# satoken/dafs

Measured on AMD Instinct MI355X. Metric: seq-pairs/sec (all-pairs ProbCons pair-HMM posteriors + sparse rows + sim), higher is better.
Workload: dtype f32; 1 GPU; N=128 L~150 synthetic random RNA (seed 12345), 8128 pairs; align_model=ProbCons, kernel=k_pairhmm3<G=32,W=6> x 4064 waves

## Files before the change

dafs_amd/capi.py:

```python
import ctypes as C
import os

import numpy as np

_HERE = os.path.dirname(os.path.abspath(__file__))
LIB_PATH = os.environ.get("DAFS_HIP_LIB") or os.path.join(_HERE, "libdafs_hip.so")

NONE = 0xFFFFFFFF
ALIGN_PROBCONS, ALIGN_CONTRALIGN = 0, 1
E_OVERFLOW = -5


class DafsHipError(RuntimeError):
    pass


def _load():
    if not os.path.exists(LIB_PATH):
        raise DafsHipError(
            "libdafs_hip.so is not built (%s). Run `python -m dafs_amd.build`; there is no CPU fallback." % LIB_PATH)
    return C.CDLL(LIB_PATH)


lib = _load()
# ... 209 lines not shown
_nodes_advance = _sig("dafs_hip_nodes_advance", C.c_int, [C.c_void_p, C.c_uint32, C.c_void_p, C.POINTER(DDParams), C.c_uint32, C.c_void_p])
_nodes_round = _sig("dafs_hip_nodes_round", C.c_int, [C.c_void_p, C.c_uint32, C.POINTER(NodeInput), C.c_void_p, C.c_uint32, C.c_void_p,
                                                      C.POINTER(DDParams), C.c_uint32, C.c_uint32, C.c_void_p, C.c_void_p])
_nodes_result = _sig("dafs_hip_nodes_result", C.c_int, [C.c_void_p, C.c_uint32, C.POINTER(NodeOutput)])
_nodes_close = _sig("dafs_hip_nodes_close", C.c_int, [C.c_void_p])
_nodes_memory = _sig("dafs_hip_nodes_memory", C.c_int, [C.c_void_p, C.POINTER(C.c_uint64), C.POINTER(C.c_uint64), C.POINTER(C.c_uint64)])
_nodes_demotions = _sig("dafs_hip_nodes_demotions", C.c_int, [C.c_void_p, C.POINTER(C.c_uint32)])
_update_basepairing = _sig("dafs_hip_update_basepairing", C.c_int, [C.c_void_p, C.c_uint32, C.c_uint32, C.c_void_p, C.c_void_p, C.c_void_p, C.c_void_p])
_consensus_structure = _sig("dafs_hip_consensus_structure", C.c_int,
                            [C.c_void_p, C.c_uint32, C.c_uint32, C.c_void_p, C.c_void_p, C.c_float, C.c_void_p,
                             C.POINTER(C.c_float), C.c_void_p])
_structure_levels_bytes = _sig("dafs_host_structure_levels_bytes", C.c_uint64, [C.c_uint32, C.c_uint32])
_consensus_structures_levels = _sig("dafs_hip_consensus_structures_levels", C.c_int,
                                    [C.c_void_p, C.c_uint32, C.c_void_p, C.c_void_p, C.c_void_p, C.c_void_p, C.c_uint32, C.c_void_p,
                                     C.c_void_p, C.c_void_p, C.c_void_p])
_structure_auto_bytes = _sig("dafs_host_structure_auto_bytes", C.c_uint64, [C.c_uint32, C.c_uint32, C.c_uint32])
_consensus_structures_auto = _sig("dafs_hip_consensus_structures_auto", C.c_int,
                                  [C.c_void_p, C.c_uint32, C.c_void_p, C.c_void_p, C.c_void_p, C.c_void_p, C.c_uint32, C.c_uint32]
                                  + [C.c_void_p] * 10)
_consensus_structures = _sig("dafs_hip_consensus_structures", C.c_int,
                             [C.c_void_p, C.c_uint32, C.c_void_p, C.c_void_p, C.c_void_p, C.c_void_p, C.c_float, C.c_void_p, C.c_void_p])
_alignment_reliability = _sig("dafs_hip_alignment_reliability", C.c_int,
                              [C.c_void_p, C.c_uint32, C.c_uint32, C.c_void_p, C.c_void_p, C.c_void_p, C.c_int, C.c_int] + [C.c_void_p] * 5)
_alignment_reliabilities = _sig("dafs_hip_alignment_reliabilities", C.c_int,
                                [C.c_void_p, C.c_uint32] + [C.c_void_p] * 6 + [C.c_int, C.c_int] + [C.c_void_p] * 5)
_alignment_covariation = _sig("dafs_hip_alignment_covariation", C.c_int,
                              [C.c_void_p, C.c_uint32, C.c_uint32, C.c_void_p, C.c_void_p, C.c_uint32, C.c_uint64] + [C.c_void_p] * 11)
_alignment_covariation_null = _sig("dafs_hip_alignment_covariation_null", C.c_int,
                                   [C.c_void_p, C.c_uint32, C.c_uint32, C.c_void_p, C.c_void_p, C.c_uint32, C.c_uint64, C.c_int, C.c_void_p,
                                    C.c_void_p] + [C.c_void_p] * 11)
_covariation_null_alignment = _sig("dafs_hip_covariation_null_alignment", C.c_int,
                                   [C.c_void_p, C.c_uint32, C.c_uint32, C.c_void_p, C.c_int, C.c_void_p, C.c_void_p, C.c_uint64, C.c_uint32,
                                    C.c_void_p])
COV_NULLS = ("shuffle", "tree")
_alignment_identity = _sig("dafs_hip_alignment_identity", C.c_int,
                           [C.c_void_p, C.c_uint32, C.c_uint32, C.c_void_p, C.c_void_p, C.c_void_p, C.c_double] + [C.c_void_p] * 7)
_alignment_weights = _sig("dafs_hip_alignment_weights", C.c_int, [C.c_void_p, C.c_uint32, C.c_uint32, C.c_void_p, C.c_void_p, C.c_void_p])


class CompareOut(C.Structure):
    _fields_ = [(k, C.c_void_p) for k in ("residues", "shared", "refp", "testp", "sps", "ppv", "total", "score", "k", "m", "colref", "colshared",
                                         "reproduced", "tc", "pair_shared", "pair_refp", "pair_testp", "pp_count", "tp", "nref", "ntest", "ss_total")]


_alignment_compare = _sig("dafs_hip_alignment_compare", C.c_int, [C.c_void_p, C.c_uint32, C.c_uint32, C.c_uint32] + [C.c_void_p] * 7 + [C.POINTER(CompareOut)])
_compare_refusal = _sig("dafs_host_compare_refusal", C.c_char_p, [C.c_int])
CMP_NEEDS_REF, CMP_NEEDS_COMPARE, CMP_NO_PAIRWISE, CMP_NEEDS_MERGED, CMP_TOO_MANY_ROWS = range(5)
_compare_match = _sig("dafs_host_compare_match", C.c_int, [C.c_uint32, C.POINTER(C.c_char_p), C.c_uint32, C.POINTER(C.c_char_p)] + [C.c_void_p] * 3)
_seed_pp = _sig("dafs_host_seed_pp", C.c_int, [C.c_char_p, C.c_size_t, C.POINTER(C.c_uint32), C.POINTER(C.c_int), C.POINTER(C.c_void_p)])
_compare_table = _sig("dafs_host_compare_table", C.c_int, [C.c_uint32, C.POINTER(C.c_char_p)] + [C.c_uint32] * 4 + [C.c_void_p] * 10 + [C.POINTER(C.c_void_p)])
_compare_columns_table = _sig("dafs_host_compare_columns_table", C.c_int, [C.c_uint32] + [C.c_void_p] * 4 + [C.POINTER(C.c_void_p)])
_compare_matrix_table = _sig("dafs_host_compare_matrix_table", C.c_int, [C.c_uint32, C.POINTER(C.c_char_p)] + [C.c_void_p] * 3 + [C.POINTER(C.c_void_p)])
_nr_select = _sig("dafs_host_nr_select", C.c_int, [C.c_uint32] + [C.c_void_p] * 5)
_ali_code = _sig("dafs_host_ali_code", C.c_uint8, [C.c_char])
_identity_summary = _sig("dafs_host_identity_summary", C.c_int, [C.c_uint32, C.c_void_p, C.c_void_p, C.c_void_p])
_identity_table = _sig("dafs_host_identity_table", C.c_int, [C.c_uint32, C.c_uint32, _strs] + [C.c_void_p] * 6 + [_text])
_identity_matrix_table = _sig("dafs_host_identity_matrix_table", C.c_int, [C.c_uint32, _strs] + [C.c_void_p] * 3 + [_text])
_stockholm_weights = _sig("dafs_host_stockholm_weights", C.c_int, [C.c_char_p, C.c_uint32, _strs, C.c_void_p, _text])
_stockholm_nr = _sig("dafs_host_stockholm_nr", C.c_int, [C.c_char_p, C.c_uint32, _strs, C.c_void_p, C.c_uint32, C.c_double, _text])
_alistat_refusal = _sig("dafs_host_alistat_refusal", C.c_char_p, [C.c_int])
NO_PAIRWISE, NR_NEEDS_MERGED, NR_THRESHOLD, TOO_MANY_ROWS = range(4)
_newick = _sig("dafs_host_newick", C.c_int, [C.c_uint32, _strs, C.c_void_p, C.c_void_p, C.c_void_p, _text])
_newick_support = _sig("dafs_host_newick_support", C.c_int, [C.c_uint32, _strs] + [C.c_void_p] * 4 + [C.c_uint32, _text])
_support_table = _sig("dafs_host_support_table", C.c_int, [C.c_uint32, _strs] + [C.c_void_p] * 3 + [C.c_uint32, C.c_uint64, C.c_int, _text])
_phylogeny_refusal = _sig("dafs_host_phylogeny_refusal", C.c_char_p, [C.c_int])
(PHY_NO_PAIRWISE, PHY_NO_SEED_EACH, PHY_TOO_MANY_ROWS, PHY_MODEL_NEEDS_TREE, PHY_UNKNOWN_MODEL, PHY_COV_TREE_NEEDS_NULL,
 PHY_UNKNOWN_COV_TREE) = range(7)
_bootstrap_refusal = _sig("dafs_host_bootstrap_refusal", C.c_char_p, [C.c_int])
BOOT_NEEDS_TREE, BOOT_COUNT, BOOT_NEEDS_REPLICATES, BOOT_NO_COLUMN = range(4)
_seed_table_nearest = _sig("dafs_host_seed_table_nearest", C.c_int, [C.c_uint32, _strs] + [C.c_void_p] * 8 + [_strs, C.c_void_p, _text])
_allgather_fn = C.CFUNCTYPE(C.c_int, C.c_void_p, C.c_void_p, C.c_void_p, C.c_size_t, C.c_void_p)
_phase1_sharded = _sig("dafs_hip_phase1_sharded", C.c_int, [C.c_void_p, C.c_uint32, C.c_uint32, C.c_int, C.c_float, C.c_float, C.c_float,
                                                           C.c_int, C.c_float, _allgather_fn, C.c_void_p])


class StageTime(C.Structure):
    _fields_ = [("kernel", C.c_char_p), ("ms", C.c_double), ("longest_ms", C.c_double), ("launches", C.c_uint32)]


_stage_timing = _sig("dafs_hip_stage_timing", C.c_int, [C.c_void_p, C.c_int])
_stage_report = _sig("dafs_hip_stage_report", C.c_int, [C.c_void_p, C.POINTER(StageTime), C.c_uint32, C.POINTER(C.c_uint32)])
pairhmm_plan = _sig("dafs_hipk_pairhmm_plan", C.c_int, [C.c_uint32, C.c_uint32, C.c_uint32, C.POINTER(PairhmmPlan)])
pairhmm3_launch = _sig("dafs_hipk_pairhmm3_launch", C.c_int, [C.POINTER(Pairhmm3Args), C.POINTER(PairhmmPlan), C.c_void_p])
pairhmm3_default_model = _sig("dafs_hip_pairhmm3_default_model", None, [C.POINTER(Pairhmm3Model)])
pairhmm5_plan = _sig("dafs_hipk_pairhmm5_plan", C.c_int, [C.c_uint32, C.c_uint32, C.c_uint32, C.POINTER(PairhmmPlan)])
pairhmm5_launch = _sig("dafs_hipk_pairhmm5_launch", C.c_int, [C.POINTER(Pairhmm5Args), C.POINTER(PairhmmPlan), C.c_void_p])
pairhmm5_default_model = _sig("dafs_hip_pairhmm5_default_model", None, [C.POINTER(Pairhmm5Model)])
residue_code = _sig("dafs_hip_residue_code", C.c_uint8, [C.c_char])
dd_node_plan = _sig("dafs_hipk_dd_node_plan", C.c_int, [C.c_uint32, C.c_uint32, C.POINTER(DdNodePlan)])
dd_lds_words = _sig("dafs_hipk_dd_lds_words", C.c_uint32, [C.c_uint32, C.c_uint32, C.c_uint32, C.c_uint32, C.c_int])


def check(rc):
    if rc != 0:
        raise DafsHipError("%s (code %d; hip: %s)" % (_strerror(rc).decode(), rc, _last_error().decode()))


def _allgather_callback(allgather, failures):
    def cb(user, send, recv, nbytes, stream):
        try:
            allgather(send, recv, nbytes)
        except BaseException as e:
            failures.append(e)
            return 1
        return 0
    return _allgather_fn(cb)


def encode(seq):
    b = seq.encode() if isinstance(seq, str) else bytes(seq)
    table = np.array([residue_code(bytes([i])) for i in range(256)], dtype=np.uint8)
    return table[np.frombuffer(b, dtype=np.uint8)]


_COV_CODE = np.array([_cov_code(bytes([i])) for i in range(256)], np.uint8)


def encode_alignment(rows):
    rows = [r.encode("latin-1") if isinstance(r, str) else bytes(r) for r in rows]
    if not rows or any(len(r) != len(rows[0]) for r in rows):
        raise ValueError("encode_alignment: at least one row, all of one length")
    return _COV_CODE[np.frombuffer(b"".join(rows), np.uint8)].reshape(len(rows), len(rows[0]))


_ALI_CODE = np.array([_ali_code(bytes([i])) for i in range(256)], np.uint8)


def encode_cells(rows):
    rows = [r.encode("latin-1") if isinstance(r, str) else bytes(r) for r in rows]
    if not rows or any(len(r) != len(rows[0]) for r in rows):
        raise ValueError("encode_cells: at least one row, all of one length")
    cell = _ALI_CODE[np.frombuffer(b"".join(rows), np.uint8)].reshape(len(rows), len(rows[0]))
    if (cell == 255).any():
        r, c = np.argwhere(cell == 255)[0]
        raise ValueError("encode_cells: row %d, column %d holds neither a letter nor a gap" % (r + 1, c + 1))
    return cell


def _cells(rows, who):
    if isinstance(rows, np.ndarray):
        if rows.ndim != 2 or rows.dtype.kind not in "iu":
            raise ValueError("%s: rows are text rows or a 2-D integer array of cells" % who)
        if rows.size and (rows.min() < 0 or rows.max() > 255):
            raise ValueError("%s: cells must fit a byte (the library refuses a code above 5)" % who)
        return np.ascontiguousarray(rows, np.uint8)
    return encode_cells(rows)


def _byte_mask(mask, size, who, what):
    if mask is None:
        return None
    mask = np.ascontiguousarray(np.asarray(mask) != 0, np.uint8)
    if mask.shape != (size,):
        raise ValueError("%s: %s" % (who, what))
    return mask


def alistat_refusal(which):
    return _alistat_refusal(which).decode()


class Identity:

    def bit(self, r, s):
        return bool((int(self.red[r, s // 32]) >> (s % 32)) & 1)

# ... 1136 lines not shown
```

dafs_amd/csrc/pair_sweeps.h:

```cpp
#pragma once
#include <hip/hip_runtime.h>
#include <stdint.h>
#include <stdlib.h>
#include "../../include/dafs_hip.h"
#include "hip_util.h"

namespace dafs {

__device__ __forceinline__ int dpp_row_shr1(int fill, int v) { return __builtin_amdgcn_update_dpp(fill, v, 0x111, 0xF, 0xF, false); }
__device__ __forceinline__ int dpp_row_shl1(int fill, int v) { return __builtin_amdgcn_update_dpp(fill, v, 0x101, 0xF, 0xF, false); }
__device__ __forceinline__ int dpp_wave_shr1(int fill, int v) { return __builtin_amdgcn_update_dpp(fill, v, 0x138, 0xF, 0xF, false); }
__device__ __forceinline__ int dpp_wave_shl1(int fill, int v) { return __builtin_amdgcn_update_dpp(fill, v, 0x130, 0xF, 0xF, false); }

template <int G>
__device__ __forceinline__ int shift_up1(int v, int fill, int t) {
  if constexpr (G == 16) return dpp_row_shr1(fill, v);
  const int r = dpp_wave_shr1(fill, v);
  if constexpr (G == 64) return r;
  return t == 0 ? fill : r;
}
template <int G>
__device__ __forceinline__ float shift_up1(float v, float fill, int t) {
  return __int_as_float(shift_up1<G>(__float_as_int(v), __float_as_int(fill), t));
}
template <int G>
__device__ __forceinline__ int shift_down1(int v, int fill, int t) {
  if constexpr (G == 16) return dpp_row_shl1(fill, v);
  const int r = dpp_wave_shl1(fill, v);
  if constexpr (G == 64) return r;
  return t == G - 1 ? fill : r;
}
template <int G>
__device__ __forceinline__ float shift_down1(float v, float fill, int t) {
  return __int_as_float(shift_down1<G>(__float_as_int(v), __float_as_int(fill), t));
}

template <int G, int W>
__device__ __forceinline__ int pair_width(int L2) {
  if constexpr (W == 1) return 1;
  int m = L2;
#pragma unroll
  for (int o = G; o < 64; o <<= 1) m = max(m, __shfl_xor(m, o));
  m = __builtin_amdgcn_readfirstlane(m);
  return (m + 1 <= G * (W - 1)) ? W - 1 : W;
}

template <int WR>
struct pair_rec {
  static constexpr int Q = (2 + WR + 3) / 4;
  static constexpr int D = 4 * Q;
};
template <int G, int W, int WR, bool dense, bool staged, class Args, class Post>
__device__ __forceinline__ bool pair_finish(const Args& a, float* __restrict__ slab, float* __restrict__ list, int list_cap, uint32_t* __restrict__ s_rowptr,
                                            uint2* __restrict__ stage, int E, int lane, int t, int g, int L1, int L2, int nsteps, bool act, uint32_t task,
                                            float th, Post post) {
  const int tlast = (L2 >= 0 ? L2 : 0) / WR;
  const int j0 = t * WR;
  typedef uint32_t u32x4 __attribute__((ext_vector_type(4)));
  const __amdgpu_buffer_rsrc_t list_rs = __builtin_amdgcn_make_buffer_rsrc((void*)list, 0, list_cap * 256, 0x00020000);
  constexpr uint32_t NO_RECORD = 0x80000000u;
  int colcnt[WR];
  float simv = 0.0f;
  uint32_t nnz = 0;
  int slab_nrec = 0;
  {
    float pdp[WR];
    int ptr[WR];
#pragma unroll
    for (int c = 0; c < WR; ++c) { pdp[c] = 0.0f; ptr[c] = 0; colcnt[c] = 0; }
    float lastdp = 0.0f, dgdp = 0.0f;
    int lasttr = 0, dgtr = 0, lastcnt = 0;
    uint32_t rowacc = 0;
    if (t == G - 1) s_rowptr[0] = 0;
    int nrec = 0;
    bool ovf = false;
    float sva[WR], svb[WR];
#pragma unroll
    for (int c = 0; c < WR; ++c) sva[c] = slab[c * 64 + lane];
#pragma unroll
    for (int c = 0; c < WR; ++c) svb[c] = slab[(W + c) * 64 + lane];
#pragma unroll
    for (int c = 0; c < WR; ++c) asm volatile("" : "+v"(sva[c]), "+v"(svb[c]));
    auto step = [&](const int s, float (&sv)[WR]) __attribute__((always_inline)) {
      const int i = s - t;
      const bool rowv = (i >= 0) && (i <= L1);
      float* __restrict__ slab_s = slab + (size_t)s * (W * 64);
      const float rdp = shift_up1<G>(lastdp, 0.0f, t);
      const int rtr = shift_up1<G>(lasttr, 0, t), rcnt = shift_up1<G>(lastcnt, 0, t);
      float ddp = dgdp, ldp = rdp;
      int dtr = dgtr, ltr = rtr, run = rcnt;
      float pp[WR];
      post(sv, pp);
      {
        const float* __restrict__ slab_n = slab + (size_t)min(s + 2, nsteps - 1) * (W * 64);
#pragma unroll
        for (int c = 0; c < WR; ++c) sv[c] = slab_n[c * 64 + lane];
      }
      uint32_t emask = 0;
#pragma unroll
      for (int c = 0; c < WR; ++c) {
        const int j = j0 + c;
        const bool v = rowv && (j <= L2);
        const bool inner = v && i >= 1 && j >= 1;
        const float p = pp[c];
        const bool entry = inner && (p >= th) && (p > th);
        if (dense) slab_s[c * 64 + lane] = entry ? p : 0.0f;
        const float udp = pdp[c];
        const int utr = ptr[c];
        const float dpe = entry ? ddp + p : -1.0f;
        const bool fl = dpe < ldp;
        float dp = fl ? ldp : dpe;
        int tr = fl ? ltr : dtr;
        const bool fu = dp < udp;
        dp = fu ? udp : dp;
        tr = (fu ? utr : tr) + 1;
        if (!inner) { dp = 0.0f; tr = 0; }
        ddp = udp; dtr = utr;
        pdp[c] = dp; ptr[c] = tr;
        ldp = dp; ltr = tr;
        const int e = entry ? 1 : 0;
        run += e;
        colcnt[c] += e;
        emask |= (uint32_t)e << c;
      }
      if (!dense) {
        const bool fits = (nrec + 1) * pair_rec<WR>::D <= list_cap;
        const bool app = emask != 0 && fits;
        ovf = ovf || (emask != 0 && !fits);
        float w[pair_rec<WR>::D];
        w[0] = __uint_as_float(emask);
        w[1] = __int_as_float((i - 1) | (rcnt << 16));
#pragma unroll
        for (int c = 0; c < WR; ++c) w[2 + c] = pp[c];
#pragma unroll
        for (int c = 2 + WR; c < pair_rec<WR>::D; ++c) w[c] = 0.0f;
        const uint32_t ro = app ? (uint32_t)(((uint32_t)nrec * pair_rec<WR>::Q * 64 + lane) * 16) : NO_RECORD;
#if !defined(PAIR_EXP_NORECSTORE)
#pragma unroll
        for (int q = 0; q < pair_rec<WR>::Q; ++q) {
          const u32x4 d = {__float_as_uint(w[4 * q]), __float_as_uint(w[4 * q + 1]), __float_as_uint(w[4 * q + 2]), __float_as_uint(w[4 * q + 3])};
          __builtin_amdgcn_raw_buffer_store_b128(d, list_rs, (int)(ro + q * 1024), 0, 0);
        }
#else
        (void)ro; (void)list_rs;
#endif
        nrec += app ? 1 : 0;
      }
      dgdp = rdp; dgtr = rtr;
      lastdp = ldp; lasttr = ltr; lastcnt = run;
      if (i == L1 && t == tlast) {
        const int cl = L2 - j0;
        float sdp = 0.0f;
        int str = 1;
#pragma unroll
        for (int c = 0; c < WR; ++c)
          if (c == cl) { sdp = pdp[c]; str = ptr[c]; }
        simv = sdp / (float)str;
      }
      if (t == G - 1 && rowv && i >= 1) {
        rowacc += (uint32_t)run;
        s_rowptr[i] = rowacc;
      }
    };
    const int nrun = dense ? nsteps : (nsteps + 1) & ~1;
    for (int s = 0; s < nrun; s += 2) {
      step(s, sva);
      if (dense && s + 1 >= nsteps) break;
      step(s + 1, svb);
    }
    nnz = rowacc;
    if (!dense && __any(ovf)) return false;
    slab_nrec = nrec;
  }
  nnz = __shfl(nnz, g * G + (G - 1));
  simv = __shfl(simv, g * G + tlast);

  int colbase[WR];
  {
    int mine = 0;
#pragma unroll
    for (int c = 0; c < WR; ++c) mine += colcnt[c];
    int incl = mine;
#pragma unroll
    for (int o = 1; o < G; o <<= 1) {
      const int up = __shfl_up(incl, o, G);
      if (t >= o) incl += up;
    }
    int run = incl - mine;
#pragma unroll
    for (int c = 0; c < WR; ++c) { colbase[c] = run; run += colcnt[c]; }
  }

#if defined(PAIR_EXP_STOP) && PAIR_EXP_STOP == 3
  if (simv != 12345.0f || nnz != 12345u || colbase[WR - 1] != 12345) return true;
#endif
  unsigned long long off = 0;
  if (t == 0 && act) off = atomicAdd(a.pool_top, 2ull * nnz);
  off = __shfl(off, g * G);
  const bool ok = act && (off + 2ull * nnz <= a.pool_cap);
  if (act && !ok && t == 0) atomicExch(a.status, DAFS_HIP_EOVERFLOW);
  const uint64_t rp = act ? a.rp_off[task] : 0;
  if (act && t == 0) {
    a.pair_off[task] = off;
    a.pair_nnz[task] = nnz;
    a.sim[task] = simv;
  }
  wave_lds_fence();
  if (act) {
    for (int r = t; r <= L1; r += G) a.rowptr_pool[rp + r] = s_rowptr[r];
    if (t == 0) a.rowptr_pool[rp + L1 + 1] = 0;
#pragma unroll
    for (int c = 0; c < WR; ++c) {
      const int j = j0 + c;
      if (j >= 1 && j <= L2) a.rowptr_pool[rp + L1 + 1 + j] = (uint32_t)(colbase[c] + colcnt[c]);
    }
  }

  if (!dense) {
    if (__any(ok)) {
      constexpr int Q = pair_rec<WR>::Q;
      constexpr int K = 4;
      int jm1 = j0 - 1;
      asm volatile("" : "+v"(jm1));
      u32x4 cur[K][Q];
      auto fetch = [&](u32x4 (&r)[K][Q], const int k0, const int n) __attribute__((always_inline)) {
#pragma unroll
        for (int kk = 0; kk < K; ++kk) {
          const uint32_t ro = (k0 + kk < n) ? (uint32_t)(((uint32_t)(k0 + kk) * Q * 64 + lane) * 16) : NO_RECORD;
#pragma unroll
          for (int q = 0; q < Q; ++q) r[kk][q] = __builtin_amdgcn_raw_buffer_load_b128(list_rs, (int)(ro + q * 1024), 0, 0);
        }
#pragma unroll
        for (int kk = 0; kk < K; ++kk)
#pragma unroll
          for (int q = 0; q < Q; ++q) asm volatile("" : "+v"(r[kk][q]));
      };
      if constexpr (!staged) {
        int maxrec = slab_nrec;
#pragma unroll
        for (int o = 1; o < 64; o <<= 1) maxrec = max(maxrec, __shfl_xor(maxrec, o));
        maxrec = __builtin_amdgcn_readfirstlane(maxrec);
        uint32_t colpos[WR];
#pragma unroll
        for (int c = 0; c < WR; ++c) colpos[c] = nnz + (uint32_t)colbase[c];
        for (int k0 = 0; k0 < maxrec; k0 += K) {
          fetch(cur, k0, slab_nrec);
#pragma unroll
          for (int kk = 0; kk < K; ++kk) {
// ... 255 lines not shown
```

dafs_amd/csrc/pairhmm3.hip:

```cpp
#include <hip/hip_runtime.h>
#include <stdint.h>
#include <stdlib.h>
#include "../../include/dafs_hip.h"
#include "pc_math.h"
#include "hip_util.h"
#include "stage.h"
#include "pair_sweeps.h"

namespace dafs {

template <int G, int W, int WR>
__device__ __forceinline__ void pairhmm3_pair(const dafs_pairhmm3_args& a, const pc_tables* tab, const float* s_match, const float* s_ins, const float2* s_mi,
                                              float* __restrict__ slab, float* __restrict__ list, int list_cap, uint32_t* __restrict__ s_rowptr, uint2* __restrict__ s_stage, int E, int lane, int t, int g,
                                              int L1, int L2, int nsteps, bool act, uint32_t task,
                                              const uint8_t* __restrict__ s1, const uint8_t* __restrict__ s2) {
  const float LZ = PC_LOG_ZERO_S;
  const float i0 = a.model.init[0], i1 = a.model.init[1], i2 = a.model.init[2];
  const float tMM = a.model.trans[0][0], tMX = a.model.trans[0][1], tMY = a.model.trans[0][2];
  const float tXM = a.model.trans[1][0], tXX = a.model.trans[1][1];
  const float tYM = a.model.trans[2][0], tYY = a.model.trans[2][2];
  const int j0 = t * WR;
  const int tlast = (L2 >= 0 ? L2 : 0) / WR;

  int cc[WR + 1];
#pragma unroll
  for (int c = 0; c <= WR; ++c) {
    const int j = j0 + c;
    cc[c] = (j >= 1 && j <= L2) ? (int)s2[j - 1] : 6;
  }
  const int c1first = act ? (int)s1[0] : 6;
  const int c2first = act ? (int)s2[0] : 6;
  const float fM11 = i0 + s_match[c1first * 8 + c2first];
  const float fX10 = i1 + s_ins[c1first];
  const float fY01 = i2 + s_ins[c2first];

  float endM = LZ, endX = LZ, endY = LZ;
  {
    float pM[WR], pX[WR], pY[WR];
#pragma unroll
    for (int c = 0; c < WR; ++c) pM[c] = pX[c] = pY[c] = LZ;
    float lastM = LZ, lastX = LZ, lastY = LZ;
    float dgM = LZ, dgX = LZ, dgY = LZ;
    int c1n = 6;
    for (int s = 0; s < nsteps; ++s) {
      const int i = s - t;
      float* __restrict__ slab_s = slab + (size_t)s * (W * 64);
      const int c1 = c1n;
      c1n = (i >= 0 && i < L1) ? (int)s1[i] : 6;
      const float rM = shift_up1<G>(lastM, LZ, t), rX = shift_up1<G>(lastX, LZ, t), rY = shift_up1<G>(lastY, LZ, t);
      const float insc1 = s_ins[c1];
      const float2* __restrict__ mi_row = s_mi + c1 * 8;
      float2 mi_prev = make_float2(0.0f, 0.0f), mi_prev2 = mi_prev;
      float m1prev = LZ, xpend = LZ;
#pragma unroll
      for (int it = 0; it < WR + 2; ++it) {
        float x[4], y[4], o[4];
#pragma unroll
        for (int n = 0; n < 4; ++n) x[n] = y[n] = LZ;
        if (it < WR) {
          const float dM = it == 0 ? dgM : pM[it > 0 ? it - 1 : 0], dX = it == 0 ? dgX : pX[it > 0 ? it - 1 : 0];
          x[0] = dM + tMM; y[0] = dX + tXM;
          x[1] = pM[it] + tMX; y[1] = pX[it] + tXX;
        }
        if (it >= 1 && it - 1 < WR) {
          const int c = it - 1;
          const float dY = c == 0 ? dgY : pY[c > 0 ? c - 1 : 0];
          x[2] = m1prev; y[2] = dY + tYM;
        }
        if (it >= 2) {
          const int c = it - 2;
          const float lM = c == 0 ? rM : pM[c > 0 ? c - 1 : 0], lY = c == 0 ? rY : pY[c > 0 ? c - 1 : 0];
          x[3] = lM + tMY; y[3] = lY + tYY;
        }
        float2 mi_now = make_float2(0.0f, 0.0f);
        if (it < WR) mi_now = mi_row[cc[it]];
        pc_log_add_n<4>(tab, x, y, o);
        if (it >= 1 && it - 1 < WR) {
          const int c = it - 1;
          float mv = o[2] + mi_prev.x;
          if (c <= 1 && s <= 2) {
            const int j = j0 + c;
            if (i <= 1 && j <= 1) mv = (i == 1 && j == 1) ? fM11 : LZ;
          }
          pM[c] = mv;
          pX[c] = xpend;
#if !defined(PAIR_EXP_NOSTORE)
          slab_s[c * 64 + lane] = mv;
#endif
        }
        if (it < WR) {
          m1prev = o[0];
          float xv = insc1 + o[1];
          if (it <= 1 && s <= 2) {
            const int j = j0 + it;
            if (i <= 1 && j <= 1) xv = (i == 1 && j == 0) ? fX10 : LZ;
          }
          xpend = xv;
// ... 45 lines not shown
      c1raw = (int)s1[max(min(nsteps - 1 - t, L1 - 1), 0)];
#pragma unroll
      for (int c = 0; c < WR; ++c) asm volatile("" : "+v"(fwd[c]));
      asm volatile("" : "+v"(c1raw));
    }
    for (int s = 0; s < nsteps; ++s) {
      const int sf = nsteps - 1 - s;
      const int i = sf - t;
      float* __restrict__ slab_s = slab + (size_t)sf * (W * 64);
      const float* __restrict__ slab_p = slab + (size_t)(sf > 0 ? sf - 1 : 0) * (W * 64);
      const int c1 = (i >= 0 && i < L1) ? c1raw : 6;
      c1raw = (int)s1[max(min(i - 1, L1 - 1), 0)];
      const float rM = shift_down1<G>(firstM, LZ, t), rY = shift_down1<G>(firstY, LZ, t);
      const float insc1 = s_ins[c1];
      const float2* __restrict__ mi_row = s_mi + c1 * 8;
      float bm1prev = LZ, by0prev = LZ, yprev = LZ, insprev = 0.0f;
      float2 mi_next = mi_row[cc[WR]];
#pragma unroll
      for (int it = 0; it < WR + 1; ++it) {
        float x[4], y[4], o[4];
        float by0now = LZ, insnow = 0.0f;
#pragma unroll
        for (int n = 0; n < 4; ++n) x[n] = y[n] = LZ;
        if (it < WR) {
          const int c = WR - 1 - it;
          const int j = j0 + c;
          const float2 mi = mi_next;
          const float dM = c == WR - 1 ? dgM : pM[c < WR - 1 ? c + 1 : 0];
          const float pxy = dM + mi.x;
          float bm = pxy + tMM, bx = pxy + tXM, by = pxy + tYM;
          if (i == L1 && j == L2) { bm = i0; bx = i1; by = i2; }
          const float tx = pX[c] + insc1;
          x[0] = bm; y[0] = tx + tMX;
          x[1] = bx; y[1] = tx + tXX;
          by0now = by;
          insnow = mi.y;
          if (c >= 1) mi_next = mi_row[cc[c]];
        }
        if (it >= 1) {
          const int c = WR - it;
          const float rgY = c == WR - 1 ? rY : yprev;
          const float ty = rgY + insprev;
          x[2] = bm1prev; y[2] = ty + tMY;
          x[3] = by0prev; y[3] = ty + tYY;
        }
        pc_log_add_n<4>(tab, x, y, o);
        if (it >= 1) {
          const int c = WR - it;
          const int j = j0 + c;
          pM[c] = o[2];
          yprev = o[3];
          slab_s[c * 64 + lane] = fwd[c] + o[2];
          fwd[c] = slab_p[c * 64 + lane];
          if (c <= 1) {
            if (i == 1 && j == 1) capM = o[2];
            if (i == 1 && j == 0) capX = pX[c];
            if (i == 0 && j == 1) capY = o[3];
          }
        }
        if (it < WR) {
          const int c = WR - 1 - it;
          bm1prev = o[0];
          by0prev = by0now;
          insprev = insnow;
          pX[c] = o[1];
        }
      }
      dgM = rM;
      firstM = pM[0];
      firstY = yprev;
    }
  }
#if defined(PAIR_EXP_STOP) && PAIR_EXP_STOP == 2
  if (capM != 12345.0f) return;
#endif
  capM = __shfl(capM, g * G + (1 / WR));
  capX = __shfl(capX, g * G);
  capY = __shfl(capY, g * G + (1 / WR));
  float totB = fM11 + capM;
  totB = pc_log_add_s(tab, totB, fX10 + capX);
  totB = pc_log_add_s(tab, totB, fY01 + capY);
  const float total = (totF + totB) / 2;

  auto post = [total, tab](const float (&sv)[WR], float (&p)[WR]) {
    float e[WR];
#pragma unroll
    for (int c = 0; c < WR; ++c) {
      const float v = (sv[c] - total) * (1.0f / PC_SCALE);
      e[c] = v < 0.0f ? v : 0.0f;
    }
    pc_exp_n<WR>(tab, e, p);
  };
  if (a.th < 0.002f || !pair_finish<G, W, WR, false, true>(a, slab, list, list_cap, s_rowptr, s_stage, E, lane, t, g, L1, L2, nsteps, act, task, a.th, post))
    (void)pair_finish<G, W, WR, true, true>(a, slab, list, list_cap, s_rowptr, s_stage, E, lane, t, g, L1, L2, nsteps, act, task, a.th, post);
}

template <int G, int W, int OCC>
__global__ __launch_bounds__(256, OCC) void k_pairhmm3(dafs_pairhmm3_args a, uint32_t slab_steps, uint32_t rp_cap, uint32_t emit_e) {
  constexpr int NG = 64 / G;
  extern __shared__ __attribute__((aligned(16))) uint32_t s_dyn[];
  __shared__ float s_match[56];
  __shared__ float s_ins[8];
  __shared__ float2 s_mi[56];
  __shared__ pc_tables s_tab;
  pc_tables_init(&s_tab, threadIdx.x);
  if (threadIdx.x < 56) s_match[threadIdx.x] = (&a.model.match[0][0])[threadIdx.x];
  if (threadIdx.x < 8) s_ins[threadIdx.x] = a.model.ins[threadIdx.x];
  if (threadIdx.x < 56) s_mi[threadIdx.x] = make_float2((&a.model.match[0][0])[threadIdx.x], a.model.ins[threadIdx.x & 7]);
  __syncthreads();
  pc_tables_init2(&s_tab, threadIdx.x, blockDim.x);
  __syncthreads();

  const int lane = threadIdx.x & 63;
  const int t = lane % G;
  const int g = lane / G;
  const int wave_in_wg = threadIdx.x >> 6;
  const uint32_t wave = __builtin_amdgcn_readfirstlane(blockIdx.x * 4 + wave_in_wg);
  const size_t plane = (size_t)slab_steps * W * 64;
  float* __restrict__ slab = a.scratch + (size_t)wave * plane * 2;
  float* __restrict__ list = slab + plane;
  const int list_cap = (int)(slab_steps * W);
  uint32_t* __restrict__ s_rowptr = s_dyn + (size_t)(wave_in_wg * NG + g) * rp_cap;
  uint2* __restrict__ s_stage = (uint2*)(s_dyn + (size_t)4 * NG * rp_cap) + (size_t)(wave_in_wg * NG + g) * (emit_e + G);

  for (;;) {
    uint32_t base = 0;
    if (lane == 0) base = atomicAdd(a.queue, (uint32_t)NG);
    base = __builtin_amdgcn_readfirstlane(base);
    if (base >= a.ntasks) break;
    const uint32_t task = base + g;
    const bool act = task < a.ntasks;
    dafs_pair_task tk = {0, 0, 0, 0};
    if (act) tk = a.tasks[task];
    const int L1 = act ? (int)tk.len1 : -1;
    const int L2 = act ? (int)tk.len2 : -1;
    const uint8_t* __restrict__ s1 = a.codes + tk.off1;
    const uint8_t* __restrict__ s2 = a.codes + tk.off2;
    int maxL1 = L1;
#pragma unroll
    for (int o = G; o < 64; o <<= 1) maxL1 = max(maxL1, __shfl_xor(maxL1, o));
    const int nsteps = __builtin_amdgcn_readfirstlane(maxL1) + G;
    if (pair_width<G, W>(L2) == W)
      pairhmm3_pair<G, W, W>(a, &s_tab, s_match, s_ins, s_mi, slab, list, list_cap, s_rowptr, s_stage, (int)emit_e, lane, t, g, L1, L2, nsteps, act, task, s1, s2);
    else
      pairhmm3_pair<G, W, (W > 1 ? W - 1 : 1)>(a, &s_tab, s_match, s_ins, s_mi, slab, list, list_cap, s_rowptr, s_stage, (int)emit_e, lane, t, g, L1, L2, nsteps, act, task, s1, s2);
  }
}

#define V(G, W, OCC) {G, W, (const void*)k_pairhmm3<G, W, OCC>, 0, OCC}
#ifdef PAIR_ONLY_VARIANTS
static pair_variant k_variants[] = {PAIR_ONLY_VARIANTS};
#else
static pair_variant k_variants[] = {
    V(16, 2, 4), V(16, 3, 4), V(16, 4, 4), V(16, 5, 4), V(16, 6, 4), V(16, 7, 3), V(16, 8, 3), V(16, 10, 2), V(16, 11, 2), V(16, 12, 2), V(16, 14, 1), V(16, 16, 1),
    V(32, 2, 4), V(32, 3, 4), V(32, 4, 4), V(32, 5, 4), V(32, 6, 4), V(32, 7, 3), V(32, 8, 3), V(32, 10, 2), V(32, 12, 2), V(32, 14, 1), V(32, 16, 1),
    V(64, 1, 4), V(64, 2, 4), V(64, 3, 4), V(64, 4, 4), V(64, 5, 4), V(64, 6, 4), V(64, 7, 3), V(64, 8, 3), V(64, 10, 2), V(64, 12, 2), V(64, 14, 1), V(64, 16, 1), V(64, 24, 1), V(64, 32, 1),
};
#endif
#undef V
static const int k_nvariants = (int)(sizeof k_variants / sizeof k_variants[0]);

}

using namespace dafs;

extern "C" int dafs_hipk_pairhmm_plan(uint32_t ntasks, uint32_t max_len1, uint32_t max_len2, dafs_pairhmm_plan* plan) {
  if (!plan || ntasks == 0 || max_len1 == 0 || max_len2 == 0) return DAFS_HIP_EINVAL;
  return pair_choose(k_variants, k_nvariants, ntasks, max_len1, max_len2, 2, 600.0, 370.0, 0.83, 0.17, plan);
}

extern "C" int dafs_hipk_pairhmm3_launch(const dafs_pairhmm3_args* args, const dafs_pairhmm_plan* plan, void* hip_stream) {
  if (!args || !plan) return DAFS_HIP_EINVAL;
  if (args->ntasks == 0) return DAFS_HIP_OK;
  pair_variant* v = nullptr;
  for (pair_variant& c : k_variants)
    if (c.G == (int)plan->group && c.W == (int)plan->width) v = &c;
  if (!v || plan->nwaves % 4 || plan->nwaves == 0) return DAFS_HIP_EINVAL;
  const uint64_t per_wave = (uint64_t)plan->slab_steps * plan->width * 64 * sizeof(float) * 2;
  if (per_wave && plan->nwaves > plan->scratch_bytes / per_wave) return DAFS_HIP_EINVAL;
  const uint32_t rp_cap = plan->slab_steps - plan->group + 1;
  const size_t rp_lds = pair_rowptr_lds(v->G, rp_cap);
  if (rp_lds > kPairRowptrLdsMax) return DAFS_HIP_ETOOLONG;
  size_t lds = 0;
  uint32_t emit_e = pair_emit_window(*v, rp_lds, &lds);
  if (lds + (size_t)v->lds_static > 64 * 1024 && !lds_optin_once(v->fn, 160 * 1024 - v->lds_static, v->optin)) return DAFS_HIP_ELAUNCH;
  dafs_pairhmm3_args a = *args;
  {
    float* f = &a.model.init[0];
    for (size_t k = 0; k < sizeof a.model / sizeof(float); ++k) f[k] *= 32.0f;
  }
  uint32_t steps = plan->slab_steps, cap = rp_cap;
  void* params[] = {&a, &steps, &cap, &emit_e};
  hipError_t launch_err = hipSuccess;
  STAGE_LAUNCH(dafs::ST_PAIRHMM3, (hipStream_t)hip_stream) launch_err = hipLaunchKernel(v->fn, dim3(plan->nwaves / 4), dim3(256), params, lds, (hipStream_t)hip_stream);
  if (hip_check(launch_err)) return DAFS_HIP_ELAUNCH;
  return DAFS_HIP_OK;
}
```

include/dafs_hip.h:

```cpp
#ifndef DAFS_HIP_H
#define DAFS_HIP_H
#include <stddef.h>
#include <stdint.h>

#ifdef __cplusplus
extern "C" {
#endif

#define DAFS_HIP_NONE 0xFFFFFFFFu

enum {
  DAFS_HIP_OK = 0,
  DAFS_HIP_EINVAL = -1,
  DAFS_HIP_ENODEV = -2,
  DAFS_HIP_ENOMEM = -3,
  DAFS_HIP_ETOOLONG = -4,
  DAFS_HIP_EOVERFLOW = -5,
  DAFS_HIP_ELAUNCH = -6,
  DAFS_HIP_ECOMM = -7
};
const char* dafs_hip_strerror(int code);
const char* dafs_hip_last_error(void);

enum { DAFS_ALIGN_PROBCONS = 0, DAFS_ALIGN_CONTRALIGN = 1 };
enum { DAFS_FOLD_CONTRAFOLD = 0 };


typedef struct {
  uint32_t off1, len1;
  uint32_t off2, len2;
} dafs_pair_task;

typedef struct {
  uint32_t group;
  uint32_t width;
  uint32_t nwaves;
  uint32_t slab_steps;
  uint64_t scratch_bytes;
} dafs_pairhmm_plan;

typedef struct {
  float init[3];
  float trans[3][3];
  float match[7][8];
  float ins[8];
} dafs_pairhmm3_model;

typedef struct {
  const uint8_t* codes;
  const dafs_pair_task* tasks;
  uint32_t ntasks;
  float th;
  float* scratch;
  uint32_t* queue;
  const uint64_t* rp_off;
  uint32_t* rowptr_pool;
  uint32_t* ent_col;
  float* ent_val;
  unsigned long long* pool_top;
  uint64_t pool_cap;
  uint64_t* pair_off;
  uint32_t* pair_nnz;
  float* sim;
  int* status;
  dafs_pairhmm3_model model;
} dafs_pairhmm3_args;

int dafs_hipk_pairhmm_plan(uint32_t ntasks, uint32_t max_len1, uint32_t max_len2, dafs_pairhmm_plan* plan);
int dafs_hipk_pairhmm3_launch(const dafs_pairhmm3_args* args, const dafs_pairhmm_plan* plan, void* hip_stream);
void dafs_hip_pairhmm3_default_model(dafs_pairhmm3_model* m);
uint8_t dafs_hip_residue_code(char c);

typedef struct {
  float match[5][5];
  float insert[5];
  float single[5];
  float pair[5][5];
} dafs_pairhmm5_model;

typedef struct {
  const uint8_t* codes;
  const dafs_pair_task* tasks;
  uint32_t ntasks;
  float th;
  float* scratch;
  uint32_t* queue;
  const uint64_t* rp_off;
  uint32_t* rowptr_pool;
  uint32_t* ent_col;
  float* ent_val;
  unsigned long long* pool_top;
  uint64_t pool_cap;
  uint64_t* pair_off;
  uint32_t* pair_nnz;
  float* sim;
  int* status;
  dafs_pairhmm5_model model;
} dafs_pairhmm5_args;

int dafs_hipk_pairhmm5_plan(uint32_t ntasks, uint32_t max_len1, uint32_t max_len2, dafs_pairhmm_plan* plan);
int dafs_hipk_pairhmm5_launch(const dafs_pairhmm5_args* args, const dafs_pairhmm_plan* plan, void* hip_stream);
void dafs_hip_pairhmm5_default_model(dafs_pairhmm5_model* m);

typedef struct dafs_hip_ctx dafs_hip_ctx;
int dafs_hip_create(int device, dafs_hip_ctx** ctx);
void dafs_hip_destroy(dafs_hip_ctx* ctx);

int dafs_hip_set_sequences(dafs_hip_ctx* ctx, uint32_t nseq, const char* const* seqs, const uint32_t* lens);
int dafs_hip_set_families(dafs_hip_ctx* ctx, uint32_t nfam, const uint32_t* first);
int dafs_hip_align_posteriors(dafs_hip_ctx* ctx, int model, float th, uint64_t pair_begin, uint64_t pair_end);
int dafs_hip_align_result_size(dafs_hip_ctx* ctx, uint64_t* npairs, uint64_t* total_nnz, uint64_t* total_rowptr);
int dafs_hip_align_fetch(dafs_hip_ctx* ctx, uint32_t* pair_x, uint32_t* pair_y, float* sim, uint32_t* nnz,
                         uint32_t* rowptr, uint32_t* col, float* val);

int dafs_hip_mp_result_size(dafs_hip_ctx* ctx, int relaxed, uint64_t* npairs, uint64_t* total_nnz, uint64_t* total_rowptr);
int dafs_hip_mp_fetch(dafs_hip_ctx* ctx, int relaxed, uint32_t* pair_x, uint32_t* pair_y, uint32_t* nnz,
                      uint32_t* rowptr, uint32_t* col, float* val);
int dafs_hip_set_mp(dafs_hip_ctx* ctx, const uint32_t* nnz, const uint32_t* rowptr, const uint32_t* col, const float* val);
int dafs_hip_mp_install(dafs_hip_ctx* ctx, int relaxed, const uint32_t* nnz, const uint32_t* rowptr, const uint32_t* col,
                        const float* val, const float* sim);
int dafs_hip_get_sim(dafs_hip_ctx* ctx, float* sim);
int dafs_hip_similarity(dafs_hip_ctx* ctx, int model, float th, uint64_t max_bytes, uint64_t* n_ranges_out);
int dafs_host_similarity_ranges(uint32_t n, const uint32_t* lens, uint64_t max_bytes, uint64_t* end, uint64_t cap, uint64_t* n_ranges);

int dafs_hip_structure_scores(dafs_hip_ctx* ctx, uint64_t* T, uint64_t* terms, uint64_t* W);
float dafs_host_structure_score(uint64_t T, uint64_t Wx, uint64_t Wy);
float dafs_host_mix_score(float sim, float str, float w);
enum { DAFS_SCORE_SEQUENCE = 0, DAFS_SCORE_STRUCTURE = 1, DAFS_SCORE_MIX = 2 };
int dafs_hip_similarity_scored(dafs_hip_ctx* ctx, int model, float th, uint64_t max_bytes, int kind, float weight, uint64_t* n_ranges_out);
int dafs_hip_get_pair_scores(dafs_hip_ctx* ctx, float* seq, float* str);

int dafs_hip_set_bp(dafs_hip_ctx* ctx, const uint32_t* rowptr, const uint32_t* col, const float* val);
int dafs_hip_bp_result_size(dafs_hip_ctx* ctx, int relaxed, uint64_t* total_nnz, uint64_t* total_rowptr);
int dafs_hip_bp_fetch(dafs_hip_ctx* ctx, int relaxed, uint32_t* rowptr, uint32_t* col, float* val);

int dafs_hip_fold_posteriors(dafs_hip_ctx* ctx, int model, float th);
int dafs_hip_fold_posteriors_begin(dafs_hip_ctx* ctx, int model, float th);
int dafs_hip_fold_posteriors_end(dafs_hip_ctx* ctx);
int dafs_hip_fold_posteriors_constrained_begin(dafs_hip_ctx* ctx, int model, float th, const char* const* constraints);
int dafs_hip_fold_posteriors_constrained(dafs_hip_ctx* ctx, int model, float th, const char* const* constraints);
int dafs_hip_fold_posteriors_levels_begin(dafs_hip_ctx* ctx, int model, float th, uint32_t nlevels, const char* const* constraints);
int dafs_hip_fold_posteriors_levels(dafs_hip_ctx* ctx, int model, float th, uint32_t nlevels, const char* const* constraints);
int dafs_hip_fold_posterior_dense(dafs_hip_ctx* ctx, const char* seq, uint32_t len, const char* constraint, float* post,
                                  float* logz);

int dafs_host_build_tree(uint32_t n, const float* sim, float* score, int32_t* left, int32_t* right);
enum { DAFS_CLUSTER_THRESHOLD = 0, DAFS_CLUSTER_COUNT = 1 };
int dafs_host_cluster_cut(uint32_t n, const float* score, const int32_t* left, const int32_t* right, int mode, float threshold,
                          uint32_t count, uint32_t* labels, uint32_t* n_clusters);

enum { DAFS_LINKAGE_SINGLE = 1, DAFS_LINKAGE_COMPLETE = 2, DAFS_LINKAGE_AVERAGE = 3 };
int dafs_hip_linkage_tree(dafs_hip_ctx* ctx, int linkage, uint32_t n, const float* sim, float* score, int32_t* left, int32_t* right);
// ... 310 lines not shown
```

Measured before the change: 6.104 million seq-pairs/s.

## Compact posterior exp evaluation across DPP lanes and skip sub-threshold cells

Adds a candidate cut in log space, log(th) minus a small margin. The few cells that exceed it are packed into fewer slots with DPP row rotations and max-reduction, so the table-based exp runs on fewer values per step. If packing collides (more candidates than packed slots), it falls back to a full exp. The exp for the next step is computed one step ahead, with a deeper slab prefetch distance, to overlap it with the sweep. This adds ballots, DPP shuffles and register pressure in exchange for fewer exp evaluations. An env var can disable the cut.

```diff
diff --git a/dafs_amd/capi.py b/dafs_amd/capi.py
--- a/dafs_amd/capi.py
+++ b/dafs_amd/capi.py
@@ -315,6 +315,7 @@
 _stage_report = _sig("dafs_hip_stage_report", C.c_int, [C.c_void_p, C.POINTER(StageTime), C.c_uint32, C.POINTER(C.c_uint32)])
 pairhmm_plan = _sig("dafs_hipk_pairhmm_plan", C.c_int, [C.c_uint32, C.c_uint32, C.c_uint32, C.POINTER(PairhmmPlan)])
 pairhmm3_launch = _sig("dafs_hipk_pairhmm3_launch", C.c_int, [C.POINTER(Pairhmm3Args), C.POINTER(PairhmmPlan), C.c_void_p])
+pairhmm3_exp_cut = _sig("dafs_hipk_pairhmm3_exp_cut", C.c_float, [C.c_float])
 pairhmm3_default_model = _sig("dafs_hip_pairhmm3_default_model", None, [C.POINTER(Pairhmm3Model)])
 pairhmm5_plan = _sig("dafs_hipk_pairhmm5_plan", C.c_int, [C.c_uint32, C.c_uint32, C.c_uint32, C.POINTER(PairhmmPlan)])
 pairhmm5_launch = _sig("dafs_hipk_pairhmm5_launch", C.c_int, [C.POINTER(Pairhmm5Args), C.POINTER(PairhmmPlan), C.c_void_p])
diff --git a/dafs_amd/csrc/pair_sweeps.h b/dafs_amd/csrc/pair_sweeps.h
--- a/dafs_amd/csrc/pair_sweeps.h
+++ b/dafs_amd/csrc/pair_sweeps.h
@@ -50,12 +50,71 @@
   static constexpr int Q = (2 + WR + 3) / 4;
   static constexpr int D = 4 * Q;
 };
+template <class Post, class = void>
+struct pair_post_cuts { static constexpr bool value = false; };
+template <class Post>
+struct pair_post_cuts<Post, decltype((void)Post::cuts)> { static constexpr bool value = true; };
+
+__device__ __forceinline__ float dpp_row_ror(float v, int n) {
+  const int i = __float_as_int(v);
+#define DAFS_ROR(N) case N: return __int_as_float(__builtin_amdgcn_update_dpp(i, i, 0x120 + N, 0xF, 0xF, true));
+  switch (n & 15) {
+    DAFS_ROR(1) DAFS_ROR(2) DAFS_ROR(3) DAFS_ROR(4) DAFS_ROR(5) DAFS_ROR(6) DAFS_ROR(7) DAFS_ROR(8)
+    DAFS_ROR(9) DAFS_ROR(10) DAFS_ROR(11) DAFS_ROR(12) DAFS_ROR(13) DAFS_ROR(14) DAFS_ROR(15)
+  }
+#undef DAFS_ROR
+  return v;
+}
+
+template <int WR>
+struct pair_passes {
+#if defined(PAIR_EXP_ONEPASS)
+  static constexpr int NP = 1, S = WR, stride = WR > 1 ? (15 / (WR - 1) < 3 ? 15 / (WR - 1) : 3) : 0;
+#else
+  static constexpr int NP = WR <= 3 ? 1 : (WR + 3) / 4;
+  static constexpr int S = (WR + NP - 1) / NP;
+  static constexpr int stride = 16 / S;
+#endif
+  static_assert(S >= 1 && (S - 1) * stride <= 15, "the slots of a pass land on distinct lanes of a row");
+};
+
+template <int WR, class Post>
+__device__ __forceinline__ bool pair_compact(const Post& post, const float (&e)[WR], float (&pp)[WR], bool (&cand)[WR]) {
+  typedef pair_passes<WR> P;
+  float acc[P::NP];
+  int ncand = 0, narrived = 0;
+#pragma unroll
+  for (int p = 0; p < P::NP; ++p) {
+#pragma unroll
+    for (int k = 0; k < P::S; ++k) {
+      const int c = p * P::S + k;
+      if (c >= WR) continue;
+      cand[c] = e[c] > post.v_cut;
+      ncand += __popcll(__ballot(cand[c]));
+      acc[p] = k == 0 ? e[c] : fmaxf(acc[p], dpp_row_ror(e[c], k * P::stride));
+    }
+    narrived += __popcll(__ballot(acc[p] > post.v_cut));
+  }
+  float pa[P::NP];
+  post.exp_all(acc, pa);
+#pragma unroll
+  for (int p = 0; p < P::NP; ++p) {
+#pragma unroll
+    for (int k = 0; k < P::S; ++k) {
+      const int c = p * P::S + k;
+      if (c >= WR) continue;
+      pp[c] = k == 0 ? pa[p] : dpp_row_ror(pa[p], 16 - k * P::stride);
+    }
+  }
+  return ncand != narrived;
+}
 template <int G, int W, int WR, bool dense, bool staged, class Args, class Post>
 __device__ __forceinline__ bool pair_finish(const Args& a, float* __restrict__ slab, float* __restrict__ list, int list_cap, uint32_t* __restrict__ s_rowptr,
                                             uint2* __restrict__ stage, int E, int lane, int t, int g, int L1, int L2, int nsteps, bool act, uint32_t task,
                                             float th, Post post) {
   const int tlast = (L2 >= 0 ? L2 : 0) / WR;
   const int j0 = t * WR;
+  constexpr bool compact = !dense && WR >= 2 && pair_post_cuts<Post>::value;
   typedef uint32_t u32x4 __attribute__((ext_vector_type(4)));
   const __amdgpu_buffer_rsrc_t list_rs = __builtin_amdgcn_make_buffer_rsrc((void*)list, 0, list_cap * 256, 0x00020000);
   constexpr uint32_t NO_RECORD = 0x80000000u;
@@ -81,6 +140,17 @@
     for (int c = 0; c < WR; ++c) svb[c] = slab[(W + c) * 64 + lane];
 #pragma unroll
     for (int c = 0; c < WR; ++c) asm volatile("" : "+v"(sva[c]), "+v"(svb[c]));
+    [[maybe_unused]] float ppn[compact ? WR : 1];
+    [[maybe_unused]] bool candn[compact ? WR : 1];
+    if constexpr (compact) {
+      float e0[WR];
+      post.arg(sva, e0);
+      const float* __restrict__ slab_n = slab + (size_t)min(2, nsteps - 1) * (W * 64);
+#pragma unroll
+      for (int c = 0; c < WR; ++c) sva[c] = slab_n[c * 64 + lane];
+      if (pair_compact<WR>(post, e0, ppn, candn)) post.exp_all(e0, ppn);
+    }
+    constexpr int AHEAD = compact ? 3 : 2;
     auto step = [&](const int s, float (&sv)[WR]) __attribute__((always_inline)) {
       const int i = s - t;
       const bool rowv = (i >= 0) && (i <= L1);
@@ -90,12 +160,22 @@
       float ddp = dgdp, ldp = rdp;
       int dtr = dgtr, ltr = rtr, run = rcnt;
       float pp[WR];
-      post(sv, pp);
+      [[maybe_unused]] bool cand[WR];
+      [[maybe_unused]] float ev[compact ? WR : 1];
+      if constexpr (compact) {
+#pragma unroll
+        for (int c = 0; c < WR; ++c) { pp[c] = ppn[c]; cand[c] = candn[c]; }
+        post.arg(sv, ev);
+      } else {
+        post(sv, pp);
+      }
       {
-        const float* __restrict__ slab_n = slab + (size_t)min(s + 2, nsteps - 1) * (W * 64);
+        const float* __restrict__ slab_n = slab + (size_t)min(s + AHEAD, nsteps - 1) * (W * 64);
 #pragma unroll
         for (int c = 0; c < WR; ++c) sv[c] = slab_n[c * 64 + lane];
       }
+      [[maybe_unused]] bool coll = false;
+      if constexpr (compact) coll = pair_compact<WR>(post, ev, ppn, candn);
       uint32_t emask = 0;
 #pragma unroll
       for (int c = 0; c < WR; ++c) {
@@ -103,7 +183,8 @@
         const bool v = rowv && (j <= L2);
         const bool inner = v && i >= 1 && j >= 1;
         const float p = pp[c];
-        const bool entry = inner && (p >= th) && (p > th);
+        bool entry = inner && (p >= th) && (p > th);
+        if constexpr (compact) entry = entry && cand[c];
         if (dense) slab_s[c * 64 + lane] = entry ? p : 0.0f;
         const float udp = pdp[c];
         const int utr = ptr[c];
@@ -161,9 +242,17 @@
         rowacc += (uint32_t)run;
         s_rowptr[i] = rowacc;
       }
+      if constexpr (compact) {
+        if (coll) post.exp_all(ev, ppn);
+      }
     };
     const int nrun = dense ? nsteps : (nsteps + 1) & ~1;
     for (int s = 0; s < nrun; s += 2) {
+      if constexpr (compact) {
+        step(s, svb);
+        step(s + 1, sva);
+        continue;
+      }
       step(s, sva);
       if (dense && s + 1 >= nsteps) break;
       step(s + 1, svb);
diff --git a/dafs_amd/csrc/pairhmm3.hip b/dafs_amd/csrc/pairhmm3.hip
--- a/dafs_amd/csrc/pairhmm3.hip
+++ b/dafs_amd/csrc/pairhmm3.hip
@@ -1,6 +1,7 @@
 #include <hip/hip_runtime.h>
 #include <stdint.h>
 #include <stdlib.h>
+#include <math.h>
 #include "../../include/dafs_hip.h"
 #include "pc_math.h"
 #include "hip_util.h"
@@ -9,10 +10,32 @@
 
 namespace dafs {
 
+template <int WR>
+struct pc_post {
+  float total;
+  const pc_tables* tab;
+  float v_cut;
+  static constexpr bool cuts = true;
+  __device__ __forceinline__ void arg(const float (&sv)[WR], float (&e)[WR]) const {
+#pragma unroll
+    for (int c = 0; c < WR; ++c) {
+      const float v = (sv[c] - total) * (1.0f / PC_SCALE);
+      e[c] = v < 0.0f ? v : 0.0f;
+    }
+  }
+  template <int N>
+  __device__ __forceinline__ void exp_all(const float (&e)[N], float (&p)[N]) const { pc_exp_n<N>(tab, e, p); }
+  __device__ __forceinline__ void operator()(const float (&sv)[WR], float (&p)[WR]) const {
+    float e[WR];
+    arg(sv, e);
+    exp_all(e, p);
+  }
+};
+
 template <int G, int W, int WR>
 __device__ __forceinline__ void pairhmm3_pair(const dafs_pairhmm3_args& a, const pc_tables* tab, const float* s_match, const float* s_ins, const float2* s_mi,
                                               float* __restrict__ slab, float* __restrict__ list, int list_cap, uint32_t* __restrict__ s_rowptr, uint2* __restrict__ s_stage, int E, int lane, int t, int g,
-                                              int L1, int L2, int nsteps, bool act, uint32_t task,
+                                              int L1, int L2, int nsteps, bool act, uint32_t task, float v_cut,
                                               const uint8_t* __restrict__ s1, const uint8_t* __restrict__ s2) {
   const float LZ = PC_LOG_ZERO_S;
   const float i0 = a.model.init[0], i1 = a.model.init[1], i2 = a.model.init[2];
@@ -224,21 +247,13 @@
   totB = pc_log_add_s(tab, totB, fY01 + capY);
   const float total = (totF + totB) / 2;
 
-  auto post = [total, tab](const float (&sv)[WR], float (&p)[WR]) {
-    float e[WR];
-#pragma unroll
-    for (int c = 0; c < WR; ++c) {
-      const float v = (sv[c] - total) * (1.0f / PC_SCALE);
-      e[c] = v < 0.0f ? v : 0.0f;
-    }
-    pc_exp_n<WR>(tab, e, p);
-  };
+  const pc_post<WR> post = {total, tab, v_cut};
   if (a.th < 0.002f || !pair_finish<G, W, WR, false, true>(a, slab, list, list_cap, s_rowptr, s_stage, E, lane, t, g, L1, L2, nsteps, act, task, a.th, post))
     (void)pair_finish<G, W, WR, true, true>(a, slab, list, list_cap, s_rowptr, s_stage, E, lane, t, g, L1, L2, nsteps, act, task, a.th, post);
 }
 
 template <int G, int W, int OCC>
-__global__ __launch_bounds__(256, OCC) void k_pairhmm3(dafs_pairhmm3_args a, uint32_t slab_steps, uint32_t rp_cap, uint32_t emit_e) {
+__global__ __launch_bounds__(256, OCC) void k_pairhmm3(dafs_pairhmm3_args a, uint32_t slab_steps, uint32_t rp_cap, uint32_t emit_e, float v_cut) {
   constexpr int NG = 64 / G;
   extern __shared__ __attribute__((aligned(16))) uint32_t s_dyn[];
   __shared__ float s_match[56];
@@ -283,9 +298,9 @@
     for (int o = G; o < 64; o <<= 1) maxL1 = max(maxL1, __shfl_xor(maxL1, o));
     const int nsteps = __builtin_amdgcn_readfirstlane(maxL1) + G;
     if (pair_width<G, W>(L2) == W)
-      pairhmm3_pair<G, W, W>(a, &s_tab, s_match, s_ins, s_mi, slab, list, list_cap, s_rowptr, s_stage, (int)emit_e, lane, t, g, L1, L2, nsteps, act, task, s1, s2);
+      pairhmm3_pair<G, W, W>(a, &s_tab, s_match, s_ins, s_mi, slab, list, list_cap, s_rowptr, s_stage, (int)emit_e, lane, t, g, L1, L2, nsteps, act, task, v_cut, s1, s2);
     else
-      pairhmm3_pair<G, W, (W > 1 ? W - 1 : 1)>(a, &s_tab, s_match, s_ins, s_mi, slab, list, list_cap, s_rowptr, s_stage, (int)emit_e, lane, t, g, L1, L2, nsteps, act, task, s1, s2);
+      pairhmm3_pair<G, W, (W > 1 ? W - 1 : 1)>(a, &s_tab, s_match, s_ins, s_mi, slab, list, list_cap, s_rowptr, s_stage, (int)emit_e, lane, t, g, L1, L2, nsteps, act, task, v_cut, s1, s2);
   }
 }
 
@@ -309,6 +324,12 @@
 extern "C" int dafs_hipk_pairhmm_plan(uint32_t ntasks, uint32_t max_len1, uint32_t max_len2, dafs_pairhmm_plan* plan) {
   if (!plan || ntasks == 0 || max_len1 == 0 || max_len2 == 0) return DAFS_HIP_EINVAL;
   return pair_choose(k_variants, k_nvariants, ntasks, max_len1, max_len2, 2, 600.0, 370.0, 0.83, 0.17, plan);
+}
+
+extern "C" float dafs_hipk_pairhmm3_exp_cut(float th) {
+  const char* e = getenv("DAFS_HIP_EXP_CUT_OFF");
+  if (e && atoi(e) != 0) return -INFINITY;
+  return logf(th) - 0.0625f;
 }
 
 extern "C" int dafs_hipk_pairhmm3_launch(const dafs_pairhmm3_args* args, const dafs_pairhmm_plan* plan, void* hip_stream) {
@@ -332,7 +353,8 @@
     for (size_t k = 0; k < sizeof a.model / sizeof(float); ++k) f[k] *= 32.0f;
   }
   uint32_t steps = plan->slab_steps, cap = rp_cap;
-  void* params[] = {&a, &steps, &cap, &emit_e};
+  float v_cut = dafs_hipk_pairhmm3_exp_cut(a.th);
+  void* params[] = {&a, &steps, &cap, &emit_e, &v_cut};
   hipError_t launch_err = hipSuccess;
   STAGE_LAUNCH(dafs::ST_PAIRHMM3, (hipStream_t)hip_stream) launch_err = hipLaunchKernel(v->fn, dim3(plan->nwaves / 4), dim3(256), params, lds, (hipStream_t)hip_stream);
   if (hip_check(launch_err)) return DAFS_HIP_ELAUNCH;
diff --git a/include/dafs_hip.h b/include/dafs_hip.h
--- a/include/dafs_hip.h
+++ b/include/dafs_hip.h
@@ -68,6 +68,7 @@
 
 int dafs_hipk_pairhmm_plan(uint32_t ntasks, uint32_t max_len1, uint32_t max_len2, dafs_pairhmm_plan* plan);
 int dafs_hipk_pairhmm3_launch(const dafs_pairhmm3_args* args, const dafs_pairhmm_plan* plan, void* hip_stream);
+float dafs_hipk_pairhmm3_exp_cut(float th);
 void dafs_hip_pairhmm3_default_model(dafs_pairhmm3_model* m);
 uint8_t dafs_hip_residue_code(char c);
 
```

Result: no change. 6.221 million seq-pairs/s (median of 3 runs) (+1.9%).
